# allenai/satlas-super-resolution

Measured on AMD Instinct MI355X. Metric: G+D train-step images/sec, higher is better.
Workload: dtype fp32h

## Files before the change

### satlas_super_resolution_amd/csrc/conv_x3r.hip

```cpp
#include "conv_x3r_core.h"

#ifdef SSR_PROBE
#define RPROBE(cond, k) do { if (cond) g_probe[(blockIdx.y * gridDim.x + blockIdx.x) * 16 + (k)] = __builtin_amdgcn_s_memtime(); } while (0)
#else
#define RPROBE(cond, k)
#endif

namespace {

template <int NTW, int NU, int EP, int TH = 8, int AM = 0>
__global__ __launch_bounds__((XrT<NTW, NU, TH>::NTHR)) void conv_x3r_kernel(const ssr_conv_desc d) {
    constexpr bool EX = AM == 1, H = AM == 2;
    using T = XrT<NTW, NU, TH>;
    constexpr int NT = NTW, NTT = T::NTT, NMF = T::NMF, BN = T::BN, WR = T::WR, MT = T::MT;
    constexpr int G_NPIX = T::NPIX, G_SUB = T::SUB, G_PV = T::PV, G_NPV = T::NPV;
    extern __shared__ __attribute__((aligned(16))) char smem[];
    int* ctl = reinterpret_cast<int*>(smem + T::CTL);
    const int ctl_addr = (int)(size_t)(__attribute__((address_space(3))) char*)(smem + T::CTL);
    const int tid = threadIdx.x, lane = tid & 63, wave = __builtin_amdgcn_readfirstlane(tid >> 6);
    const int tiles_x = (d.Gw + 15) / 16, tiles_y = (d.Gh + TH - 1) / TH;
    int b = blockIdx.x;
    const int tx_i = b % tiles_x; b /= tiles_x;
    const int ty_i = b % tiles_y;
    const int n = b / tiles_y;
    const int gy0 = ty_i * TH, gx0 = tx_i * 16;
    const int co0 = blockIdx.y * BN;
    const int Cin = d.Cin, Cin2 = d.Cin2;
    const int nchunks = (Cin + Cin2 + 15) / 16;
    const int cout_pad = d.CoutPad;
    const int tapstride = cout_pad * 64, wchunk = 9 * tapstride;
    RPROBE(tid == 0, 0);
    if (tid < 4 + NMF) ctl[tid] = 0;
    __syncthreads();

    f32x16 acc[MT][NT];
#pragma unroll
    for (int t = 0; t < MT; ++t)
#pragma unroll
        for (int u = 0; u < NT; ++u)
#pragma unroll
            for (int r = 0; r < 16; ++r) acc[t][u][r] = 0.f;

    if (wave >= NMF) {
        const int pw = wave - NMF;
        const int pt = tid - 64 * NMF;
#ifdef XR_PRIO
        __builtin_amdgcn_s_setprio(3);
#endif
        const int part = pt & 3, p4 = pt >> 2;
        int ppix[G_NPV];
#pragma unroll
        for (int q = 0; q < G_NPV; ++q) {
            const int pix = p4 + 64 * q;
            const int py = pix / XR_PW, px = pix - py * XR_PW;
            const int ly = gy0 + py - d.pad_y, lx = gx0 + px - d.pad_x;
            const bool okp = pix < G_NPIX && ly >= 0 && ly < d.Hi && lx >= 0 && lx < d.Wi;
            ppix[q] = okp ? (n * d.Hi + ly) * d.Wi + lx : -1;
        }
        const int plo0 = p4 * XR_ROWB + part * 8;
        const long xbytes = (long)d.N * d.Hi * d.Wi * 4;
        const void* xp = d.x.p;
        const void* x2p = d.x2.p ? d.x2.p : d.x.p;
        const int x_cs = d.x.cs, x_coff = d.x.coff, x2_cs = d.x2.p ? d.x2.cs : d.x.cs, x2_coff = d.x2.p ? d.x2.coff : d.x.coff;
        u32x4 rq[XR_PQ][G_NPV];
        auto load_chunk = [&](int c, auto jc) {
            constexpr int j = decltype(jc)::value;
            const bool live = c < nchunks;
            const int c0 = c * 16;
            const bool in_x = c0 < Cin;
            const int cb = in_x ? c0 : c0 - Cin, clim = live ? (in_x ? Cin : Cin2) : 0;
            const int cs = in_x ? x_cs : x2_cs, coff = in_x ? x_coff : x2_coff;
            const __amdgpu_buffer_rsrc_t rs = xr_rsrc(in_x ? xp : x2p, xbytes * cs);
            const int k = cb + part * 4;
#pragma unroll
            for (int q = 0; q < G_NPV; ++q) {
                const int off = (ppix[q] * cs + coff + k) * 4;
                const bool okl = (k < clim) & (ppix[q] >= 0);
#ifdef XR_X_NOXLOAD
                rq[j][q] = u32x4{(unsigned)off, (unsigned)okl, 0u, 0u};
#else
                rq[j][q] = __builtin_amdgcn_raw_buffer_load_b128(rs, okl ? off : XR_OOB, 0, 0);
#endif
            }
        };
        static_for<0, XR_PQ>([&](auto jc) { __builtin_amdgcn_sched_barrier(0); load_chunk(decltype(jc)::value, jc); __builtin_amdgcn_sched_barrier(0); });
        RPROBE(pt == 0, 8);
        int cfree = XR_NS;
        for (int c0 = 0; c0 < nchunks; c0 += XR_PQ) {
            static_for<0, XR_PQ>([&](auto jc) {
                constexpr int j = decltype(jc)::value;
                const int c = c0 + j;
                if (c < nchunks) {
                    if (c >= cfree) {
                        int spin = 0;
                        for (; spin < XR_SPIN_MAX; ++spin) {
                            cfree = xr_minN<NMF>(ctl_addr + 16) + XR_NS;
                            if (c < cfree) break;
                            __builtin_amdgcn_s_sleep(2);
                        }
                        if (spin == XR_SPIN_MAX) __builtin_trap();
                    }
                    char* base = smem + (c % XR_NS) * G_SUB;
#pragma unroll
                    for (int q = 0; q < G_NPV; ++q) {
#ifdef XR_X_NOSTORE
                        asm volatile("" :: "v"(rq[j][q]));
                        continue;
#endif
                        if constexpr (EX) {
                            if (q < G_NPV - 1 || pt < G_PV - (G_NPV - 1) * 256)
                                *reinterpret_cast<u32x4*>(base + p4 * XR_ROWB + part * 16 + q * 64 * XR_ROWB) = rq[j][q];
                        } else {
                            uint2 hi, lo;
                            split_f32x4<H>(rq[j][q], hi, lo);
                            if (q < G_NPV - 1 || pt < G_PV - (G_NPV - 1) * 256) {
                                *reinterpret_cast<uint2*>(base + plo0 + q * 64 * XR_ROWB) = hi;
                                *reinterpret_cast<uint2*>(base + plo0 + q * 64 * XR_ROWB + 32) = lo;
                            }
                        }
                    }
                    asm volatile("" ::: "memory");
                    if (lane == 0) *(xr_lds_int)(uintptr_t)(ctl_addr + 4 * pw) = c + 1;
                    asm volatile("" ::: "memory");
#if defined(XR_PRIO) && XR_PRIO == 1
                    if (c == 0) __builtin_amdgcn_s_setprio(0);
#endif
                }
                __builtin_amdgcn_sched_barrier(0);
                load_chunk(c + XR_PQ, jc);
                __builtin_amdgcn_sched_barrier(0);
            });
        }
        RPROBE(pt == 0, 9);
    } else {
        const int w = wave & 3, ug = wave >> 2;
        const int i = lane & 31, gq = lane >> 5;
        const int a_lane = ((i >> 4) * XR_PW + epi_col<XR_ROT>(i)) * XR_ROWB + gq * 16;
        const __amdgpu_buffer_rsrc_t rsw = xr_rsrc(d.w, (long)nchunks * wchunk);
        const int w_lane = (co0 + 32 * NTW * ug + i) * 64 + gq * 16;
        const int nitems = 3 * nchunks;
        const int nj = nitems > w ? (nitems - w + 3) / 4 : 0;
        const int glast = w + 4 * (nj - 1);
        if (nj == 0) {
            if (lane == 0) *(xr_lds_int)(uintptr_t)(ctl_addr + 16 + 4 * wave) = 0x3fffffff;
        } else {
            bf16x8 wf[WR][NT][2];
            constexpr int TPS = T::TPS, SPT = T::SPT, NSUB = 3 * SPT, NSETS = T::NSETS, PD = NSETS - 1;
            bf16x8 af[NSETS][TPS][2];
            auto load_w = [&](int g_, auto kxc, auto sc) {
                constexpr int kx = decltype(kxc)::value, s = decltype(sc)::value;
                const int gg = g_ < glast ? g_ : glast;
                const int c = gg / 3, ky = gg - 3 * c;
                const int off = c * wchunk + (ky * 3 + kx) * tapstride + w_lane;
#pragma unroll
                for (int u = 0; u < NT; ++u) {
                    wf[s][u][0] = __builtin_bit_cast(bf16x8, __builtin_amdgcn_raw_buffer_load_b128(rsw, off + u * 2048, 0, 0));
                    wf[s][u][1] = __builtin_bit_cast(bf16x8, __builtin_amdgcn_raw_buffer_load_b128(rsw, off + u * 2048 + 32, 0, 0));
                }
            };
            auto issue_a = [&](int base, auto qc, auto sc, auto hc) {
                constexpr int q = decltype(qc)::value, kx = q / SPT, part = q % SPT, s = decltype(sc)::value, H = decltype(hc)::value;
#pragma unroll
                for (int t2 = 0; t2 < TPS; ++t2)
                    af[s][t2][H] = *reinterpret_cast<const bf16x8*>(smem + base + kx * XR_ROWB + (part * TPS + t2) * XR_TILEB + 32 * H);
            };
            int avail = 0;
            auto ensure = [&](int c) {
                if (avail > c) return;
                int spin = 0;
                for (; spin < XR_SPIN_MAX; ++spin) {
                    avail = xr_min4(ctl_addr);
                    if (avail > c) break;
                    __builtin_amdgcn_s_sleep(1);
                }
                if (spin == XR_SPIN_MAX) __builtin_trap();
            };
            auto base_of = [&](int g_) { const int c = g_ / 3, ky = g_ - 3 * c; return (c % XR_NS) * G_SUB + ky * XR_PW * XR_ROWB + a_lane; };
            using I0 = std::integral_constant<int, 0>;
            using I1 = std::integral_constant<int, 1>;
#ifndef XR_WPRE
#define XR_WPRE 99
#endif
            constexpr int WPRE = XR_WPRE < WR ? XR_WPRE : WR;
            static_for<0, WPRE>([&](auto sc) {
                constexpr int s = decltype(sc)::value;
                __builtin_amdgcn_sched_barrier(0);
                load_w(w + 4 * (s / 3), std::integral_constant<int, s % 3>{}, sc);
                __builtin_amdgcn_sched_barrier(0);
            });
            RPROBE(tid == 0, 1);
            int g = w, c_cur = g / 3;
            int base_cur = base_of(g);
            ensure(c_cur);
            static_for<WPRE, WR>([&](auto sc) {
                constexpr int s = decltype(sc)::value;
                __builtin_amdgcn_sched_barrier(0);
                load_w(w + 4 * (s / 3), std::integral_constant<int, s % 3>{}, sc);
                __builtin_amdgcn_sched_barrier(0);
            });
            RPROBE(tid == 0, 2);
            static_for<0, PD>([&](auto qc) {
                issue_a(base_cur, qc, std::integral_constant<int, decltype(qc)::value % NSETS>{}, I1{});
                issue_a(base_cur, qc, std::integral_constant<int, decltype(qc)::value % NSETS>{}, I0{});
            });
            int gn = g + 4 < glast ? g + 4 : glast;
            int c_next = gn / 3, base_next = base_of(gn);
            int gnn = gn, c_nn = c_next, base_nn = base_next;
            auto body = [&](int j, auto jpc) {
                constexpr int JP = decltype(jpc)::value;
                static_for<0, NSUB>([&](auto qc) {
                    constexpr int q = decltype(qc)::value, kx = q / SPT, part = q % SPT, qn = q + PD;
                    constexpr int ws = (JP * 3 + kx) % WR, as = (JP * NSUB + q) % NSETS, asn = (JP * NSUB + qn) % NSETS;
                    auto group = [&](auto pc) {
                        constexpr int P = decltype(pc)::value;
                        if constexpr (EX) {
                            constexpr int H = P == 0 ? 1 : 0, S0 = P == 2 ? 2 : 0, S1 = P == 1 ? 2 : 4;
#pragma unroll
                            for (int sidx = S0; sidx < S1; ++sidx)
#pragma unroll
                                for (int t2 = 0; t2 < TPS; ++t2)
#pragma unroll
                                    for (int u = 0; u < NT; ++u) {
                                        const f32x4 av = __builtin_bit_cast(f32x4, af[as][t2][H]), bv = __builtin_bit_cast(f32x4, wf[ws][u][H]);
                                        acc[part * TPS + t2][u] = __builtin_amdgcn_mfma_f32_32x32x2f32(av[sidx], bv[sidx], acc[part * TPS + t2][u], 0, 0, 0);
                                    }
                        } else {
#pragma unroll
                            for (int t2 = 0; t2 < TPS; ++t2)
#pragma unroll
                                for (int u = 0; u < NT; ++u)
                                    acc[part * TPS + t2][u] = split_mfma<H>(af[as][t2][P == 0 ? 1 : 0], wf[ws][u][P == 1 ? 1 : 0], acc[part * TPS + t2][u]);
                        }
                    };
                    auto reads = [&](auto hc) {
#ifndef XR_X_NOA
                        if constexpr (qn < NSUB) issue_a(base_cur, std::integral_constant<int, qn>{}, std::integral_constant<int, asn>{}, hc);
                        else issue_a(base_next, std::integral_constant<int, qn - NSUB>{}, std::integral_constant<int, asn>{}, hc);
#endif
                    };
                    __builtin_amdgcn_sched_barrier(0);
                    if constexpr (qn == NSUB) {
                        if (c_next > c_cur) {
                            asm volatile("" ::: "memory");
                            if (lane == 0) *(xr_lds_int)(uintptr_t)(ctl_addr + 16 + 4 * wave) = c_next;
                            asm volatile("" ::: "memory");
                        }
                        ensure(c_next);
                        __builtin_amdgcn_sched_barrier(0);
                    }
                    group(std::integral_constant<int, 0>{});
                    __builtin_amdgcn_sched_barrier(0);
                    reads(I1{});
                    if constexpr (part == 0) {
#ifndef XR_X_NOW
                        constexpr int wsp = (JP * 3 + kx + WR - 1) % WR, ioff = (kx + WR - 1) / 3, tap = (kx + WR - 1) % 3;
                        load_w(g + 4 * ioff, std::integral_constant<int, tap>{}, std::integral_constant<int, wsp>{});
#endif
                    }
                    __builtin_amdgcn_sched_barrier(0);
                    group(std::integral_constant<int, 1>{});
                    __builtin_amdgcn_sched_barrier(0);
                    reads(I0{});
                    if constexpr (q == 0) {
                        gnn = g + 8 < glast ? g + 8 : glast;
                        c_nn = gnn / 3;
                        base_nn = base_of(gnn);
                    }
                    __builtin_amdgcn_sched_barrier(0);
                    group(std::integral_constant<int, 2>{});
                    __builtin_amdgcn_sched_barrier(0);
                });
                g += 4;
                c_cur = c_next; base_cur = base_next;
                gn = gnn; c_next = c_nn; base_next = base_nn;
#ifdef SSR_PROBE
                if (j < 5) RPROBE(tid == 0, 3 + j);
#endif
            };
            if constexpr (WR == 6 || (NSUB % NSETS) != 0) {
                for (int j = 0; j < nj; j += 2) {
                    body(j, std::integral_constant<int, 0>{});
                    if (j + 1 < nj) body(j + 1, std::integral_constant<int, 1>{});
                }
            } else {
                for (int j = 0; j < nj; ++j) body(j, std::integral_constant<int, 0>{});
            }
            asm volatile("" ::: "memory");
            if (lane == 0) *(xr_lds_int)(uintptr_t)(ctl_addr + 16 + 4 * wave) = 0x3fffffff;
        }
    }
    __syncthreads();
    RPROBE(tid == 0, 10);

    const bool is_mfma = wave < NMF;
    const int me = is_mfma ? (wave & 3) : wave - NMF;
    const int ut = is_mfma ? NTW * (wave >> 2) : 1;
#ifndef XR_X_NORED
    if (is_mfma) {
#pragma unroll
        for (int t = 0; t < MT; ++t)
#pragma unroll
            for (int u = 0; u < NT; ++u)
                if (!(t == me && u == 0)) {
                    char* sp = smem + ((me * MT + t) * NTT + ut + u) * XR_SLOT + lane * 16;
#pragma unroll
                    for (int q = 0; q < 4; ++q) {
                        f32x4 v = {acc[t][u][4 * q], acc[t][u][4 * q + 1], acc[t][u][4 * q + 2], acc[t][u][4 * q + 3]};
                        *reinterpret_cast<f32x4*>(sp + q * 1024) = v;
                    }
                }
    }
#endif
    __syncthreads();
    if ((is_mfma || NTW == 2) && me < MT) {
        f32x16 own;
#pragma unroll
        for (int r = 0; r < 16; ++r) own[r] = 0.f;
        if (is_mfma) {
#pragma unroll
            for (int t = 0; t < MT; ++t)
                if (t == me) own = acc[t][0];
        }
        f32x16 sum;
#pragma unroll
        for (int s = 0; s < 4; ++s) {
            f32x16 part;
            const char* sp = smem + ((s * MT + me) * NTT + ut) * XR_SLOT + lane * 16;
#ifdef XR_X_NORED
            part = own;
            asm volatile("" : "+v"(part));
#else
#pragma unroll
            for (int q = 0; q < 4; ++q) {
                const f32x4 v = *reinterpret_cast<const f32x4*>(sp + q * 1024);
                part[4 * q] = v[0]; part[4 * q + 1] = v[1]; part[4 * q + 2] = v[2]; part[4 * q + 3] = v[3];
            }
#endif
            const bool mine = is_mfma && s == me;
#pragma unroll
            for (int r = 0; r < 16; ++r) {
                const float p = mine ? own[r] : part[r];
                sum[r] = s == 0 ? p : sum[r] + p;
            }
        }
        if constexpr (H) {
#pragma unroll
            for (int r = 0; r < 16; ++r) sum[r] *= SSR_F32H_UNSCALE;
        }
        char* slab = smem + (((is_mfma ? me : 0) * MT + me) * NTT + ut) * XR_SLOT;
        const int cb = co0 + 32 * ut;
#ifdef XR_X_NOEPI
        float keep = 0.f;
#pragma unroll
        for (int r = 0; r < 16; ++r) keep += sum[r];
        if (keep == 123.456f) reinterpret_cast<float*>(d.y.p)[tid] = keep;
#else
        if constexpr (EP == XR_EP_GENERIC) conv_epilogue<float, XR_ROT>(d, sum, cb, n, gy0 + 2 * me, gx0, lane, slab);
        else xr_epilogue<EP>(d, sum, cb, n, gy0 + 2 * me, gx0, lane, slab);
#endif
    }
    RPROBE(tid == 0, 11);
}

template <int NTW, int NU, int EP, int TH = 8, int AM = 0>
int launch_x3r(const ssr_conv_desc& d, hipStream_t st) {
    using T = XrT<NTW, NU, TH>;
    auto kern = conv_x3r_kernel<NTW, NU, EP, TH, AM>;
    static bool attr_done[SSR_MAX_DEVICES] = {};
    const int dev = ssr_device_ordinal();
    if (!attr_done[dev]) {
        hipError_t e = hipFuncSetAttribute(reinterpret_cast<const void*>(kern), hipFuncAttributeMaxDynamicSharedMemorySize, T::LDS);
        if (e != hipSuccess) return (int)e;
        attr_done[dev] = true;
    }
    const int tiles = ((d.Gw + 15) / 16) * ((d.Gh + TH - 1) / TH) * d.N;
    hipLaunchKernelGGL(kern, dim3(tiles, d.CoutPad / T::BN, 1), dim3(T::NTHR), T::LDS, st, d);
    SSR_LAUNCH_CHECK();
    return SSR_OK;
}

int xr_pick_epilogue(const ssr_conv_desc& d) {
    static const bool generic_only = [] { const char* e = getenv("SSR_X3R_EPI"); return e && e[0] == '0'; }();
    if (generic_only) return XR_EP_GENERIC;
    const long lim = 0x7fffff00L, npx = (long)d.N * d.Ho * d.Wo * 4;
    auto vok = [&](const ssr_view& v) { return (v.cs % 4) == 0 && (v.coff % 4) == 0 && ((uintptr_t)v.p % 16) == 0 && npx * v.cs <= lim; };
    if (d.fix_list || d.y0.p || d.y1.p || d.accumulate || d.m_relu || (d.Cout % 4) != 0 || !vok(d.y)) return XR_EP_GENERIC;
    if (d.oys != 1 || d.oxs != 1 || d.oyo != 0 || d.oxo != 0 || d.Ho < d.Gh || d.Wo < d.Gw) return XR_EP_GENERIC;
    const bool r1 = d.r1.p != nullptr, r2 = d.r2.p != nullptr, m = d.m.p != nullptr;
    if (d.act == SSR_ACT_LRELU && d.alpha == 1.f && !r1 && !r2 && !m) return XR_EP_LRELU;
    if (d.act == SSR_ACT_NONE && !m && (!r1 || (d.r1_nc >= d.Cout && vok(d.r1))) && (!r2 || (d.r2_nc >= d.Cout && vok(d.r2)))) return XR_EP_LIN;
    if (d.act == SSR_ACT_NONE && d.alpha == 1.f && m && !r1 && !r2 && d.m_c0 == 0 && d.m_c1 >= d.Cout && vok(d.m)) return XR_EP_MASK;
    return XR_EP_GENERIC;
}

template <int NTW, int NU, int TH = 8, int AM = 0>
int launch_x3r_ep(const ssr_conv_desc& d, hipStream_t st) {
    switch (xr_pick_epilogue(d)) {
        case XR_EP_LRELU: return launch_x3r<NTW, NU, XR_EP_LRELU, TH, AM>(d, st);
        case XR_EP_LIN: return launch_x3r<NTW, NU, XR_EP_LIN, TH, AM>(d, st);
        case XR_EP_MASK: return launch_x3r<NTW, NU, XR_EP_MASK, TH, AM>(d, st);
        default: return launch_x3r<NTW, NU, XR_EP_GENERIC, TH, AM>(d, st);
    }
}

int xr_tile_height(const ssr_conv_desc& d, int form) {
    static const int forced = [] { const char* e = getenv("SSR_X3_REGTILE_TH"); return e ? atoi(e) : 0; }();
    if (form != 0) return 8;
    if (forced == 4 || forced == 8) return forced;
    const long tiles8 = (long)((d.Gw + 15) / 16) * ((d.Gh + 7) / 8) * d.N * (d.CoutPad / 32);
    return (tiles8 <= 160 && d.Gh > 4) ? 4 : 8;
}

int xr_wide_form(const ssr_conv_desc& d) {
    static const int f = [] { const char* e = getenv("SSR_X3_REGTILE_NT2"); return !e ? 1 : e[0] == '0' ? 0 : e[0] == '8' ? 2 : 1; }();
    if ((d.CoutPad % 64) != 0) return 0;
    static const bool split_off = [] { const char* e = getenv("SSR_X3_REGTILE_SPLIT"); return e && e[0] == '0'; }();
    const long tiles = (long)((d.Gw + 15) / 16) * ((d.Gh + 7) / 8) * d.N;
    if (!split_off && tiles * (d.CoutPad / 64) <= 160) return 0;
    return (f == 2 && xr_pick_epilogue(d) == XR_EP_GENERIC) ? 1 : f;
}

}

void ssr_conv_x3r_instance(const ssr_conv_desc& d, int* ntw, int* nu, int* ep) {
    int f = xr_wide_form(d);
    if ((d.dtype == SSR_F32 || d.dtype == SSR_F32H) && f == 2) f = 1;
    *ntw = f == 1 ? 2 : 1;
    *nu = f == 2 ? 2 : 1;
    *ep = xr_pick_epilogue(d);
}
int ssr_conv_x3r_tile_height(const ssr_conv_desc& d) { return xr_tile_height(d, xr_wide_form(d)); }

bool ssr_conv_x3r_shape_ok(const ssr_conv_desc& d) {
    static const bool ex_off = [] { const char* e = getenv("SSR_F32_REGTILE"); return e && e[0] == '0'; }();
    if (!(d.dtype == SSR_F32X3 || d.dtype == SSR_F32H || (d.dtype == SSR_F32 && !ex_off)) || d.fix_list) return false;
    if (d.dtype == SSR_F32 && (d.act == SSR_ACT_RELU || d.m_relu)) return false;
    if (!(d.KH == 3 && d.KW == 3 && d.stride == 1 && d.pad_y == 1 && d.pad_x == 1 && d.up == 1 && !d.s2d)) return false;
    if (d.Gh != d.Hi || d.Gw != d.Wi || (d.CoutPad % 32) != 0) return false;
    if (d.x2.p && (d.Cin % 16) != 0) return false;
    const long lim = 0x7fffff00L, npx = (long)d.N * d.Hi * d.Wi * 4;
    if (npx * d.x.cs > lim || (d.x2.p && npx * d.x2.cs > lim)) return false;
    if ((long)((d.Cin + d.Cin2 + 15) / 16) * 9 * d.CoutPad * 64 > lim) return false;
    return true;
}

bool ssr_conv_x3r_qualifies(const ssr_conv_desc& d) {
    static const bool off = [] { const char* e = getenv("SSR_X3_REGTILE"); return e && e[0] == '0'; }();
    if (off || !ssr_conv_x3r_shape_ok(d)) return false;
    return d.Gh <= 64 && d.Gw <= 64 && d.Cin + d.Cin2 >= 16;
}

bool ssr_conv_x3r_try(const ssr_conv_desc& d, hipStream_t st, int* rc, bool force) {
    if (force ? !ssr_conv_x3r_shape_ok(d) : !ssr_conv_x3r_qualifies(d)) return false;
    const int f = xr_wide_form(d);
    if (d.dtype == SSR_F32) {
        if (f != 0) *rc = launch_x3r_ep<2, 1, 8, 1>(d, st);
        else *rc = xr_tile_height(d, f) == 4 ? launch_x3r_ep<1, 1, 4, 1>(d, st) : launch_x3r_ep<1, 1, 8, 1>(d, st);
        return true;
    }
    if (d.dtype == SSR_F32H) {
        if (f != 0) *rc = launch_x3r_ep<2, 1, 8, 2>(d, st);
        else *rc = xr_tile_height(d, f) == 4 ? launch_x3r_ep<1, 1, 4, 2>(d, st) : launch_x3r_ep<1, 1, 8, 2>(d, st);
        return true;
    }
    if (f == 2) *rc = launch_x3r_ep<1, 2>(d, st);
    else if (f == 1) *rc = launch_x3r_ep<2, 1>(d, st);
    else *rc = xr_tile_height(d, f) == 4 ? launch_x3r_ep<1, 1, 4>(d, st) : launch_x3r_ep<1, 1, 8>(d, st);
    return true;
}
```

### satlas_super_resolution_amd/csrc/conv_x3r_core.h

```cpp
#pragma once
#include "conv_epilogue.h"
#include <cstdlib>

namespace {

constexpr int XR_NMFMA = 4, XR_NPROD = 4, XR_NTHR = 64 * (XR_NMFMA + XR_NPROD);
constexpr int XR_ROWB = 80, XR_PH = 10, XR_PW = 18, XR_NPIX = XR_PH * XR_PW;
constexpr int XR_SUB = XR_NPIX * XR_ROWB;
constexpr int XR_NS = 8;
constexpr int XR_RING = XR_NS * XR_SUB;
constexpr int XR_PV = XR_NPIX * 4;
constexpr int XR_NPV = (XR_PV + 255) / 256;
#ifndef XR_PQ_DEPTH
#define XR_PQ_DEPTH 4
#endif
constexpr int XR_PQ = XR_PQ_DEPTH;
constexpr int XR_ROT = 14;
constexpr int XR_OOB = 0x7ffffff0;
constexpr int XR_SPIN_MAX = 1 << 22;
constexpr int XR_TILEB = 2 * XR_PW * XR_ROWB;
constexpr int XR_SLOT = 32 * 32 * 4;

template <int NTW, int NU = 1, int TH = 8> struct XrT {
    static_assert(TH == 8 || TH == 4, "tile height");
    static constexpr int MT = TH / 2;
    static constexpr int PH = TH + 2, NPIX = PH * XR_PW;
    static constexpr int SUB = NPIX * XR_ROWB;
    static constexpr int RING = XR_NS * SUB;
    static constexpr int PV = NPIX * 4, NPV = (PV + 255) / 256;
    static constexpr int NTT = NTW * NU;
    static constexpr int BN = 32 * NTT;
    static constexpr int NMF = 4 * NU;
    static constexpr int NTHR = 64 * (NMF + 4);
    static constexpr int WR = (NTW == 1 && NU == 1) ? 6 : 3;
#ifndef XR_TPS1
#define XR_TPS1 4
#endif
    static constexpr int TPS = (NTW == 1 ? XR_TPS1 : 2) < MT ? (NTW == 1 ? XR_TPS1 : 2) : MT;
    static constexpr int SPT = MT / TPS;
    static constexpr int NSETS = SPT == 1 ? 2 : 3;
    static constexpr int SLOTS = 4 * MT * NTT;
    static constexpr int RED = SLOTS * XR_SLOT;
    static constexpr int CTL = RED > RING ? RED : RING;
    static constexpr int LDS = CTL + 256;
    static_assert(LDS <= 160 * 1024, "LDS budget");
};

__device__ __forceinline__ __amdgpu_buffer_rsrc_t xr_rsrc(const void* p, long bytes) {
    return __builtin_amdgcn_make_buffer_rsrc(const_cast<void*>(p), 0, (int)(bytes > 0x7fffff00L ? 0x7fffff00L : (bytes < 0 ? 0 : bytes)), 0x00020000);
}
__device__ __forceinline__ void xr_split4(const u32x4& v, uint2& hi, uint2& lo) {
    const f32x4 f = __builtin_bit_cast(f32x4, v);
    bf16x4 h, l;
#pragma unroll
    for (int k = 0; k < 4; ++k) {
        h[k] = (__bf16)f[k];
        l[k] = (__bf16)(f[k] - (float)h[k]);
    }
    hi = __builtin_bit_cast(uint2, h);
    lo = __builtin_bit_cast(uint2, l);
}
typedef __attribute__((address_space(3))) int* xr_lds_int;

__device__ __forceinline__ int xr_min4(int a) {
    u32x4 v;
    asm volatile("ds_read_b128 %0, %1\n\ts_waitcnt lgkmcnt(0)" : "=&v"(v) : "v"(a) : "memory");
    return __builtin_amdgcn_readfirstlane((int)min(min(v[0], v[1]), min(v[2], v[3])));
}

template <int N> __device__ __forceinline__ int xr_minN(int a) {
    if constexpr (N == 4) return xr_min4(a);
    else {
        u32x4 v, w;
        asm volatile("ds_read_b128 %0, %2\n\tds_read_b128 %1, %2 offset:16\n\ts_waitcnt lgkmcnt(0)" : "=&v"(v), "=&v"(w) : "v"(a) : "memory");
        const unsigned m = min(min(min(v[0], v[1]), min(v[2], v[3])), min(min(w[0], w[1]), min(w[2], w[3])));
        return __builtin_amdgcn_readfirstlane((int)m);
    }
}

enum { XR_EP_LRELU = 0, XR_EP_LIN = 1, XR_EP_MASK = 2, XR_EP_GENERIC = 3 };

template <int EP, int AUX = 0>
__device__ __forceinline__ void xr_epilogue(const ssr_conv_desc& d, const f32x16& acc, int co_base, int n, int gy_row0, int gx0, int lane,
                                             char* slab) {
    const int i = lane & 31, g = lane >> 5;
    const int part = lane & 7, c = co_base + part * 4;
    const bool cok = c < d.Cout;
    const long npix = (long)d.N * d.Ho * d.Wo * 4;
    const __amdgpu_buffer_rsrc_t rs_y = xr_rsrc(d.y.p, npix * d.y.cs);
    int pp[4];
    bool ok[4];
#pragma unroll
    for (int h = 0; h < 4; ++h) {
        const int pix = (lane >> 3) + 8 * h;
        const int gy = gy_row0 + (pix >> 4), gx = gx0 + epi_col<XR_ROT>(pix);
        ok[h] = cok && gy < d.Gh && gx < d.Gw;
        pp[h] = (n * d.Ho + gy) * d.Wo + gx;
    }
    f32x4 bv = {0.f, 0.f, 0.f, 0.f};
    if (d.bias) {
        const __amdgpu_buffer_rsrc_t rs_b = xr_rsrc(d.bias, (long)d.Cout * 4);
#pragma unroll
        for (int k = 0; k < 4; ++k) bv[k] = __builtin_bit_cast(float, __builtin_amdgcn_raw_buffer_load_b32(rs_b, (c + k) * 4, 0, 0));
    }
    u32x4 q1[4], q2[4];
    if constexpr (EP == XR_EP_LIN) {
        const __amdgpu_buffer_rsrc_t rs_r1 = xr_rsrc(d.r1.p, d.r1.p ? npix * d.r1.cs : 0), rs_r2 = xr_rsrc(d.r2.p, d.r2.p ? npix * d.r2.cs : 0);
        const bool h1 = d.r1.p != nullptr, h2 = d.r2.p != nullptr;
#pragma unroll
        for (int h = 0; h < 4; ++h) {
            q1[h] = __builtin_amdgcn_raw_buffer_load_b128(rs_r1, ok[h] && h1 ? (pp[h] * d.r1.cs + d.r1.coff + c) * 4 : XR_OOB, 0, 0);
            q2[h] = __builtin_amdgcn_raw_buffer_load_b128(rs_r2, ok[h] && h2 ? (pp[h] * d.r2.cs + d.r2.coff + c) * 4 : XR_OOB, 0, 0);
        }
    }
    if constexpr (EP == XR_EP_MASK) {
        const __amdgpu_buffer_rsrc_t rs_m = xr_rsrc(d.m.p, npix * d.m.cs);
#pragma unroll
        for (int h = 0; h < 4; ++h) q1[h] = __builtin_amdgcn_raw_buffer_load_b128(rs_m, ok[h] ? (pp[h] * d.m.cs + d.m.coff + c) * 4 : XR_OOB, 0, 0);
    }
    float* sl = reinterpret_cast<float*>(slab);
#pragma unroll
    for (int r = 0; r < 16; ++r) sl[mfma32_row(r, g) * 32 + i] = acc[r];
    const float alpha = d.alpha, beta1 = d.beta1, beta2 = d.beta2;
#pragma unroll
    for (int h = 0; h < 4; ++h) {
        const int pix = (lane >> 3) + 8 * h;
        f32x4 v = *reinterpret_cast<const f32x4*>(sl + pix * 32 + part * 4);
        if constexpr (EP == XR_EP_LRELU) {
#pragma unroll
            for (int k = 0; k < 4; ++k) v[k] = lrelu_max(v[k] + bv[k]);
        } else if constexpr (EP == XR_EP_LIN) {
            const f32x4 a = __builtin_bit_cast(f32x4, q1[h]), b = __builtin_bit_cast(f32x4, q2[h]);
#pragma unroll
            for (int k = 0; k < 4; ++k) v[k] = alpha * (v[k] + bv[k]) + (beta1 * a[k] + beta2 * b[k]);
        } else {
            const f32x4 m = __builtin_bit_cast(f32x4, q1[h]);
#pragma unroll
            for (int k = 0; k < 4; ++k) v[k] = (v[k] + bv[k]) * lrelu_grad_from_out(m[k]);
        }
        __builtin_amdgcn_raw_buffer_store_b128(__builtin_bit_cast(u32x4, v), rs_y, ok[h] ? (pp[h] * d.y.cs + d.y.coff + c) * 4 : XR_OOB, 0, AUX);
    }
}

}
```

Before: 1166.

## Use 3D grid, defer entry barrier, split epilogue across producer waves

```diff
diff --git a/satlas_super_resolution_amd/csrc/conv_x3r.hip b/satlas_super_resolution_amd/csrc/conv_x3r.hip
--- a/satlas_super_resolution_amd/csrc/conv_x3r.hip
+++ b/satlas_super_resolution_amd/csrc/conv_x3r.hip
@@ -1,12 +1,28 @@
 #include "conv_x3r_core.h"
 
 #ifdef SSR_PROBE
-#define RPROBE(cond, k) do { if (cond) g_probe[(blockIdx.y * gridDim.x + blockIdx.x) * 16 + (k)] = __builtin_amdgcn_s_memtime(); } while (0)
+#define RPROBE(cond, k) do { if (cond) g_probe[((blockIdx.z * gridDim.y + blockIdx.y) * gridDim.x + blockIdx.x) * 16 + (k)] = __builtin_amdgcn_s_memtime(); } while (0)
 #else
 #define RPROBE(cond, k)
 #endif
 
+#ifndef XR_GRID3
+#define XR_GRID3 1
+#endif
+#ifndef XR_LATEBAR
+#define XR_LATEBAR 1
+#endif
+#ifndef XR_EPI8
+#define XR_EPI8 1
+#endif
+
 namespace {
+
+__device__ __forceinline__ void xr_entry_barrier() {
+#if XR_LATEBAR
+    asm volatile("s_waitcnt lgkmcnt(0)\n\ts_barrier" ::: "memory");
+#endif
+}
 
 template <int NTW, int NU, int EP, int TH = 8, int AM = 0>
 __global__ __launch_bounds__((XrT<NTW, NU, TH>::NTHR)) void conv_x3r_kernel(const ssr_conv_desc d) {
@@ -18,20 +34,29 @@
     int* ctl = reinterpret_cast<int*>(smem + T::CTL);
     const int ctl_addr = (int)(size_t)(__attribute__((address_space(3))) char*)(smem + T::CTL);
     const int tid = threadIdx.x, lane = tid & 63, wave = __builtin_amdgcn_readfirstlane(tid >> 6);
+#if XR_GRID3
+    const int tx_i = blockIdx.x, ty_i = blockIdx.y;
+    int n = blockIdx.z, cblk = 0;
+    while (n >= d.N) { n -= d.N; ++cblk; }
+#else
     const int tiles_x = (d.Gw + 15) / 16, tiles_y = (d.Gh + TH - 1) / TH;
     int b = blockIdx.x;
     const int tx_i = b % tiles_x; b /= tiles_x;
     const int ty_i = b % tiles_y;
     const int n = b / tiles_y;
+    const int cblk = blockIdx.y;
+#endif
     const int gy0 = ty_i * TH, gx0 = tx_i * 16;
-    const int co0 = blockIdx.y * BN;
+    const int co0 = cblk * BN;
     const int Cin = d.Cin, Cin2 = d.Cin2;
     const int nchunks = (Cin + Cin2 + 15) / 16;
     const int cout_pad = d.CoutPad;
     const int tapstride = cout_pad * 64, wchunk = 9 * tapstride;
     RPROBE(tid == 0, 0);
     if (tid < 4 + NMF) ctl[tid] = 0;
+#if !XR_LATEBAR
     __syncthreads();
+#endif
 
     f32x16 acc[MT][NT];
 #pragma unroll
@@ -83,8 +108,14 @@
 #endif
             }
         };
-        static_for<0, XR_PQ>([&](auto jc) { __builtin_amdgcn_sched_barrier(0); load_chunk(decltype(jc)::value, jc); __builtin_amdgcn_sched_barrier(0); });
+        static_for<0, XR_PQ>([&](auto jc) {
+            __builtin_amdgcn_sched_barrier(0);
+            load_chunk(decltype(jc)::value, jc);
+            __builtin_amdgcn_sched_barrier(0);
+            if constexpr (decltype(jc)::value == 0) RPROBE(pt == 0, 13);
+        });
         RPROBE(pt == 0, 8);
+        xr_entry_barrier();
         int cfree = XR_NS;
         for (int c0 = 0; c0 < nchunks; c0 += XR_PQ) {
             static_for<0, XR_PQ>([&](auto jc) {
@@ -142,6 +173,7 @@
         const int nj = nitems > w ? (nitems - w + 3) / 4 : 0;
         const int glast = w + 4 * (nj - 1);
         if (nj == 0) {
+            xr_entry_barrier();
             if (lane == 0) *(xr_lds_int)(uintptr_t)(ctl_addr + 16 + 4 * wave) = 0x3fffffff;
         } else {
             bf16x8 wf[WR][NT][2];
@@ -187,8 +219,10 @@
                 __builtin_amdgcn_sched_barrier(0);
                 load_w(w + 4 * (s / 3), std::integral_constant<int, s % 3>{}, sc);
                 __builtin_amdgcn_sched_barrier(0);
+                if constexpr (s == 0) RPROBE(tid == 0, 12);
             });
             RPROBE(tid == 0, 1);
+            xr_entry_barrier();
             int g = w, c_cur = g / 3;
             int base_cur = base_of(g);
             ensure(c_cur);
@@ -295,24 +329,65 @@
     const bool is_mfma = wave < NMF;
     const int me = is_mfma ? (wave & 3) : wave - NMF;
     const int ut = is_mfma ? NTW * (wave >> 2) : 1;
+#if XR_EPI8 && !defined(XR_X_NORED) && !defined(XR_X_NOEPI)
+    constexpr bool SPLIT = NTW == 1 && NU == 1 && EP != XR_EP_GENERIC;
+#else
+    constexpr bool SPLIT = false;
+#endif
+    const int q0 = is_mfma ? 0 : 2;
 #ifndef XR_X_NORED
     if (is_mfma) {
 #pragma unroll
         for (int t = 0; t < MT; ++t)
 #pragma unroll
             for (int u = 0; u < NT; ++u)
-                if (!(t == me && u == 0)) {
+                if (SPLIT || !(t == me && u == 0)) {
                     char* sp = smem + ((me * MT + t) * NTT + ut + u) * XR_SLOT + lane * 16;
 #pragma unroll
                     for (int q = 0; q < 4; ++q) {
                         f32x4 v = {acc[t][u][4 * q], acc[t][u][4 * q + 1], acc[t][u][4 * q + 2], acc[t][u][4 * q + 3]};
-                        *reinterpret_cast<f32x4*>(sp + q * 1024) = v;
+                        if (!SPLIT || q >= 2 || t != me) *reinterpret_cast<f32x4*>(sp + q * 1024) = v;
                     }
                 }
     }
 #endif
     __syncthreads();
-    if ((is_mfma || NTW == 2) && me < MT) {
+    if constexpr (SPLIT) {
+        if (me < MT) {
+            float own[8], sum[8];
+#pragma unroll
+            for (int r = 0; r < 8; ++r) own[r] = 0.f;
+            if (is_mfma) {
+#pragma unroll
+                for (int t = 0; t < MT; ++t)
+                    if (t == me) {
+#pragma unroll
+                        for (int r = 0; r < 8; ++r) own[r] = acc[t][0][r];
+                    }
+            }
+#pragma unroll
+            for (int s = 0; s < 4; ++s) {
+                float part[8];
+                const char* sp = smem + (s * MT + me) * XR_SLOT + q0 * 1024 + lane * 16;
+#pragma unroll
+                for (int q = 0; q < 2; ++q) {
+                    const f32x4 v = *reinterpret_cast<const f32x4*>(sp + q * 1024);
+                    part[4 * q] = v[0]; part[4 * q + 1] = v[1]; part[4 * q + 2] = v[2]; part[4 * q + 3] = v[3];
+                }
+                const bool mine = is_mfma && s == me;
+#pragma unroll
+                for (int r = 0; r < 8; ++r) {
+                    const float p = mine ? own[r] : part[r];
+                    sum[r] = s == 0 ? p : sum[r] + p;
+                }
+            }
+            if constexpr (H) {
+#pragma unroll
+                for (int r = 0; r < 8; ++r) sum[r] *= SSR_F32H_UNSCALE;
+            }
+            xr_epilogue<EP, 0, 2>(d, sum, co0, n, gy0 + 2 * me, gx0, lane, smem + (me * MT + me) * XR_SLOT, q0);
+        }
+    } else if ((is_mfma || NTW == 2) && me < MT) {
         f32x16 own;
 #pragma unroll
         for (int r = 0; r < 16; ++r) own[r] = 0.f;
@@ -373,8 +448,13 @@
         if (e != hipSuccess) return (int)e;
         attr_done[dev] = true;
     }
+#if XR_GRID3
+    if ((long)d.N * (d.CoutPad / T::BN) > 65535) return SSR_EUNSUP;
+    hipLaunchKernelGGL(kern, dim3((d.Gw + 15) / 16, (d.Gh + TH - 1) / TH, d.N * (d.CoutPad / T::BN)), dim3(T::NTHR), T::LDS, st, d);
+#else
     const int tiles = ((d.Gw + 15) / 16) * ((d.Gh + TH - 1) / TH) * d.N;
     hipLaunchKernelGGL(kern, dim3(tiles, d.CoutPad / T::BN, 1), dim3(T::NTHR), T::LDS, st, d);
+#endif
     SSR_LAUNCH_CHECK();
     return SSR_OK;
 }
diff --git a/satlas_super_resolution_amd/csrc/conv_x3r_core.h b/satlas_super_resolution_amd/csrc/conv_x3r_core.h
--- a/satlas_super_resolution_amd/csrc/conv_x3r_core.h
+++ b/satlas_super_resolution_amd/csrc/conv_x3r_core.h
@@ -80,19 +80,19 @@
 
 enum { XR_EP_LRELU = 0, XR_EP_LIN = 1, XR_EP_MASK = 2, XR_EP_GENERIC = 3 };
 
-template <int EP, int AUX = 0>
-__device__ __forceinline__ void xr_epilogue(const ssr_conv_desc& d, const f32x16& acc, int co_base, int n, int gy_row0, int gx0, int lane,
-                                             char* slab) {
+template <int EP, int AUX = 0, int NQ = 4, class ACC>
+__device__ __forceinline__ void xr_epilogue(const ssr_conv_desc& d, const ACC& acc, int co_base, int n, int gy_row0, int gx0, int lane,
+                                             char* slab, int q0 = 0) {
     const int i = lane & 31, g = lane >> 5;
     const int part = lane & 7, c = co_base + part * 4;
     const bool cok = c < d.Cout;
     const long npix = (long)d.N * d.Ho * d.Wo * 4;
     const __amdgpu_buffer_rsrc_t rs_y = xr_rsrc(d.y.p, npix * d.y.cs);
-    int pp[4];
-    bool ok[4];
+    int pp[NQ];
+    bool ok[NQ];
 #pragma unroll
-    for (int h = 0; h < 4; ++h) {
-        const int pix = (lane >> 3) + 8 * h;
+    for (int h = 0; h < NQ; ++h) {
+        const int pix = (lane >> 3) + 8 * (q0 + h);
         const int gy = gy_row0 + (pix >> 4), gx = gx0 + epi_col<XR_ROT>(pix);
         ok[h] = cok && gy < d.Gh && gx < d.Gw;
         pp[h] = (n * d.Ho + gy) * d.Wo + gx;
@@ -103,12 +103,12 @@
 #pragma unroll
         for (int k = 0; k < 4; ++k) bv[k] = __builtin_bit_cast(float, __builtin_amdgcn_raw_buffer_load_b32(rs_b, (c + k) * 4, 0, 0));
     }
-    u32x4 q1[4], q2[4];
+    u32x4 q1[NQ], q2[NQ];
     if constexpr (EP == XR_EP_LIN) {
         const __amdgpu_buffer_rsrc_t rs_r1 = xr_rsrc(d.r1.p, d.r1.p ? npix * d.r1.cs : 0), rs_r2 = xr_rsrc(d.r2.p, d.r2.p ? npix * d.r2.cs : 0);
         const bool h1 = d.r1.p != nullptr, h2 = d.r2.p != nullptr;
 #pragma unroll
-        for (int h = 0; h < 4; ++h) {
+        for (int h = 0; h < NQ; ++h) {
             q1[h] = __builtin_amdgcn_raw_buffer_load_b128(rs_r1, ok[h] && h1 ? (pp[h] * d.r1.cs + d.r1.coff + c) * 4 : XR_OOB, 0, 0);
             q2[h] = __builtin_amdgcn_raw_buffer_load_b128(rs_r2, ok[h] && h2 ? (pp[h] * d.r2.cs + d.r2.coff + c) * 4 : XR_OOB, 0, 0);
         }
@@ -116,14 +116,14 @@
     if constexpr (EP == XR_EP_MASK) {
         const __amdgpu_buffer_rsrc_t rs_m = xr_rsrc(d.m.p, npix * d.m.cs);
 #pragma unroll
-        for (int h = 0; h < 4; ++h) q1[h] = __builtin_amdgcn_raw_buffer_load_b128(rs_m, ok[h] ? (pp[h] * d.m.cs + d.m.coff + c) * 4 : XR_OOB, 0, 0);
+        for (int h = 0; h < NQ; ++h) q1[h] = __builtin_amdgcn_raw_buffer_load_b128(rs_m, ok[h] ? (pp[h] * d.m.cs + d.m.coff + c) * 4 : XR_OOB, 0, 0);
     }
-    float* sl = reinterpret_cast<float*>(slab);
+    float* sl = reinterpret_cast<float*>(slab) + q0 * 8 * 32;
 #pragma unroll
-    for (int r = 0; r < 16; ++r) sl[mfma32_row(r, g) * 32 + i] = acc[r];
+    for (int r = 0; r < 4 * NQ; ++r) sl[mfma32_row(r, g) * 32 + i] = acc[r];
     const float alpha = d.alpha, beta1 = d.beta1, beta2 = d.beta2;
 #pragma unroll
-    for (int h = 0; h < 4; ++h) {
+    for (int h = 0; h < NQ; ++h) {
         const int pix = (lane >> 3) + 8 * h;
         f32x4 v = *reinterpret_cast<const f32x4*>(sl + pix * 32 + part * 4);
         if constexpr (EP == XR_EP_LRELU) {
```

Result: no change. 1177, median of 6 (+1.0%).
